# kaist-cvml/3d-vlm-gd

Hardware: AMD Instinct MI355X
Metric: image-pairs/sec (518^2, ViT-B/14 LoRA) student distillation step (higher is better)
Workload: dtype tf32h; 1 GPU; finetune_timm_mast3r_objaverse: vit_base/14 + LoRA(r=4,q,v)+adapters blocks 4-11, 518^2 pairs, shared-518 geometry, mast3r losses (AP+depth+intra+cost-KL), 32 pairs/GPU, 300 keypoints/pair, hw=1369; pairs_per_gpu=32, global_pairs=32, parallelism=dp1, world_size_seen=1, backend=nccl (RCCL), exchange=torch, engine_dtype=tf32h

## Files before the change

### 3d-vlm-gd_amd/_lib.py

```python
import ctypes
import os

_HERE = os.path.dirname(os.path.abspath(__file__))
LIB_PATH = os.environ.get("GD_HIP_LIB") or os.path.join(_HERE, "lib", "libgd_hip.so")
_lib = None

F32, BF16, F16 = 0, 1, 3
MATCH_COLS = 1

c_int, c_long, c_float, c_void_p, c_size_t = ctypes.c_int, ctypes.c_long, ctypes.c_float, ctypes.c_void_p, ctypes.c_size_t

ABI_VERSION = 4
SIGNATURES = {
    "gd_last_error": (ctypes.c_char_p, []),
    "gd_abi_version": (c_int, []),
    "gd_debug_set": (c_int, [ctypes.c_char_p, c_int]),
    "gd_debug_get": (c_int, [ctypes.c_char_p]),
    "gd_gemm_phase_probe": (c_int, [c_int, c_void_p]),
    "gd_loss_combine_fwd": (c_int, [c_void_p, c_void_p, c_void_p, c_void_p, ctypes.POINTER(c_float), c_void_p, c_int, c_void_p, c_void_p, c_void_p]),
    "gd_loss_combine_bwd": (c_int, [c_void_p, ctypes.POINTER(c_float), c_void_p, c_int, c_void_p, c_void_p]),
    "gd_depth_bwd_combine": (c_int, [c_void_p, c_void_p, c_void_p, c_void_p, c_void_p, c_void_p, c_int, c_int, c_int, c_void_p, c_void_p, c_void_p]),
    "gd_scale_and_transpose": (c_int, [c_void_p, c_void_p, c_void_p, c_void_p, c_int, c_int, c_int, c_void_p]),
    "gd_gemm_nt": (c_int, [c_void_p, c_void_p, c_void_p, c_int, c_int, c_int, c_long, c_long, c_long,
                           c_int, c_long, c_long, c_long, c_int, c_int, c_float,
# ... 10 lines not shown
                                           c_int, c_int, c_int, c_int, c_void_p, c_void_p, c_void_p, c_void_p]),
    "gd_cost_volume_kl_bwd_rows_workspace_bytes": (c_size_t, [c_int, c_int, c_int, c_int, c_int]),
    "gd_cost_volume_kl_bwd_rows": (c_int, [c_void_p, c_void_p, c_void_p, c_void_p, c_void_p, c_void_p, c_int, c_void_p, c_void_p, c_int, c_int, c_int,
                                           c_int, c_int, c_void_p, c_void_p, c_void_p, c_void_p, c_void_p, c_void_p]),
    "gd_cost_volume_kl_bwd_h_workspace_bytes": (c_size_t, [c_int, c_int, c_int]),
    "gd_cost_volume_kl_bwd_h": (c_int, [c_void_p, c_void_p, c_void_p, c_void_p, c_void_p, c_void_p, c_int, c_void_p, c_void_p, c_int, c_int, c_int,
                                        c_void_p, c_void_p, c_void_p, c_void_p, c_void_p, c_void_p]),
    "gd_gemm_nt_copy16": (c_int, [c_void_p, c_void_p, c_void_p, c_int, c_int, c_int, c_long, c_long, c_long, c_float, c_void_p, c_void_p,
                                  c_void_p, c_long, c_void_p, c_long, c_void_p, c_void_p]),
    "gd_tap_mean_norm_fwd_h": (c_int, [c_void_p, c_int, c_long, c_int, c_void_p, c_void_p, c_void_p, c_int, c_int, c_int, c_void_p]),
    "gd_adapter_fused_h_supported": (c_int, [c_int, c_int, c_long]),
    "gd_adapter_fused_h_ln": (c_int, [c_void_p, c_void_p, c_void_p, c_void_p, c_void_p, c_void_p, c_void_p, c_float, c_void_p, c_void_p, c_void_p,
                                      c_int, c_int, c_int, c_void_p]),
    "gd_adapter_fused_h": (c_int, [c_void_p, c_void_p, c_void_p, c_void_p, c_void_p, c_void_p, c_void_p, c_void_p, c_void_p, c_void_p,
                                   c_int, c_int, c_int, c_void_p]),
    "gd_gemm_tn_scaled": (c_int, [c_void_p, c_void_p, c_void_p, c_int, c_int, c_int, c_long, c_long, c_long,
                                  c_int, c_long, c_long, c_long, c_int, c_int, c_float, c_void_p, c_void_p]),
    "gd_cast_f16": (c_int, [c_void_p, c_void_p, c_long, c_int, c_long, c_float, c_void_p, c_void_p]),
    "gd_amax_scale": (c_int, [c_void_p, c_long, c_int, c_long, c_float, c_void_p, c_void_p, c_void_p]),
    "gd_scale_from_amax": (c_int, [c_void_p, c_float, c_void_p, c_void_p]),
    "gd_cast_f16_ex": (c_int, [c_void_p, c_void_p, c_long, c_int, c_long, c_float, c_void_p, c_void_p, c_void_p]),
    "gd_layernorm_bwd_ex": (c_int, [c_void_p, c_int, c_void_p, c_void_p, c_void_p, c_void_p, c_void_p, c_void_p, c_void_p, c_void_p, c_void_p, c_void_p,
                                    c_void_p, c_void_p, c_int, c_int, c_long, c_long, c_float, c_void_p]),
    "gd_gemm_tn": (c_int, [c_void_p, c_void_p, c_void_p, c_int, c_int, c_int, c_long, c_long, c_long,
                           c_int, c_long, c_long, c_long, c_int, c_int, c_float, c_void_p]),
    "gd_layernorm_fwd": (c_int, [c_void_p, c_void_p, c_void_p, c_void_p, c_void_p, c_void_p, c_int, c_int, c_long,
                                 c_long, c_float, c_int, c_int, c_void_p]),
    "gd_layernorm_bwd": (c_int, [c_void_p, c_void_p, c_void_p, c_void_p, c_void_p, c_void_p, c_void_p, c_void_p, c_int, c_int,
                                 c_long, c_long, c_float, c_int, c_int, c_void_p]),
    "gd_adapter_fused_supported": (c_int, [c_int, c_int, c_int]),
    "gd_adapter_fused": (c_int, [c_void_p, c_void_p, c_void_p, c_void_p, c_void_p, c_void_p, c_int, c_int, c_int, c_int,
                                 c_void_p]),
    "gd_l2norm_fwd": (c_int, [c_void_p, c_void_p, c_void_p, c_int, c_int, c_float, c_void_p]),
    "gd_l2norm_bwd": (c_int, [c_void_p, c_void_p, c_void_p, c_void_p, c_int, c_int, c_void_p]),
    "gd_patch_im2col": (c_int, [c_void_p, c_void_p, c_int, c_int, c_int, c_int, c_int, c_int, c_int,
                                ctypes.POINTER(c_float), ctypes.POINTER(c_float), c_int, c_void_p]),
    "gd_patch_im2col_strided": (c_int, [c_void_p, c_void_p, c_int, c_int, c_int, c_int, c_int, c_int, c_int, c_int, c_int,
                                        ctypes.POINTER(c_float), ctypes.POINTER(c_float), c_int, c_void_p]),
    "gd_assemble_tokens": (c_int, [c_void_p, c_void_p, c_void_p, c_void_p, c_int, c_int, c_int, c_int, c_void_p]),
    "gd_im2col3x3": (c_int, [c_void_p, c_long, c_void_p, c_int, c_int, c_int, c_int, c_int, c_void_p]),
    "gd_col2im3x3": (c_int, [c_void_p, c_void_p, c_long, c_int, c_int, c_int, c_int, c_int, c_void_p]),
    "gd_kp_gather_fwd": (c_int, [ctypes.POINTER(c_void_p), c_int, c_long, c_int, c_void_p, c_void_p, c_int, c_int,
                                 c_int, c_int, c_int, c_float, c_float, c_int, c_int, c_int, c_int, c_int, c_void_p]),
    "gd_kp_gather_fwd_ln": (c_int, [ctypes.POINTER(c_void_p), ctypes.POINTER(c_void_p), ctypes.POINTER(c_void_p), c_int, c_long, c_long, c_int, c_void_p, c_void_p,
                                    c_void_p, c_void_p, c_int, c_int, c_int, c_int, c_int, c_float, c_float, c_int, c_int, c_int, c_int, c_int, c_void_p]),
    "gd_kp_gather_bwd": (c_int, [ctypes.POINTER(c_void_p), c_int, c_long, c_void_p, c_void_p, c_int, c_int, c_int, c_int,
# ... 156 lines not shown
```

### 3d-vlm-gd_amd/csrc/norm.hip

```cpp
#include "gd_common.h"
#include <stdlib.h>

#define LN_MAXV 8

template <typename T> __device__ __forceinline__ f32x4 load4(const T* p);
template <> __device__ __forceinline__ f32x4 load4<float>(const float* p) { return *(const f32x4*)p; }
template <> __device__ __forceinline__ f32x4 load4<bf16>(const bf16* p) {
    const bf16x4 v = *(const bf16x4*)p;
    return f32x4{(float)v[0], (float)v[1], (float)v[2], (float)v[3]};
}
template <typename T> __device__ __forceinline__ void store4n(T* p, f32x4 v);
template <> __device__ __forceinline__ void store4n<float>(float* p, f32x4 v) { *(f32x4*)p = v; }
template <> __device__ __forceinline__ void store4n<bf16>(bf16* p, f32x4 v) {
    *(bf16x4*)p = bf16x4{(bf16)v[0], (bf16)v[1], (bf16)v[2], (bf16)v[3]};
}
template <> __device__ __forceinline__ void store4n<f16>(f16* p, f32x4 v) {
    *(f16x4*)p = f16_sat4(v[0], v[1], v[2], v[3]);
}

template <typename T, typename TO, int NV>
__global__ __launch_bounds__(256) void ln_fwd_kernel(const T* x, const float* gamma, const float* beta, TO* y,
                                                     float* mean, float* rstd, int M, int D, long ldx, long ldy,
                                                     float eps) {
    const int lane = threadIdx.x & 63, row = blockIdx.x * 4 + (threadIdx.x >> 6);
// ... 32 lines not shown
            for (int k = 0; k < 4; ++k) o[k] = (v[i][k] - mu) * rs * g[k] + b[k];
            store4n<TO>(yr + c, o);
        }
    }
}

template <> __device__ __forceinline__ f32x4 load4<f16>(const f16* p) {
    const f16x4 v = *(const f16x4*)p;
    return f32x4{(float)v[0], (float)v[1], (float)v[2], (float)v[3]};
}
__device__ __forceinline__ unsigned wave_umax(unsigned v) {
#pragma unroll
    for (int o = 32; o > 0; o >>= 1) { const unsigned w = (unsigned)__shfl_xor((int)v, o, 64); v = w > v ? w : v; }
    return v;
}
__device__ __forceinline__ unsigned wave_uadd(unsigned v) {
#pragma unroll
    for (int o = 32; o > 0; o >>= 1) v += (unsigned)__shfl_xor((int)v, o, 64);
    return v;
}
#define GD_AMAX_SLOTS 256
#define GD_RANGE_SLOTS 64

template <typename T, typename TD, int NV>
__global__ __launch_bounds__(256) void ln_bwd_kernel(const TD* dy, const T* x, const float* gamma, const float* mean,
                                                     const float* rstd, const T* dres, const T* dres2, T* dx, int M, int D,
                                                     long ldd, long ldx, float dyscale, f16* dx16 = nullptr, const float* sdev = nullptr,
                                                     const float* dys_dev = nullptr, unsigned* amax = nullptr, unsigned* range = nullptr) {
    const int lane = threadIdx.x & 63;
    int row = blockIdx.x * 4 + (threadIdx.x >> 6);
    const bool live = row < M;
    if (!live) {
        if (!amax && !range) return;
        row = M - 1;
    }
    const float mu = mean[row], rs = rstd[row];
    const float s16 = (dx16 && sdev) ? *sdev : 1.0f;
    if (dys_dev) dyscale *= *dys_dev;
    const T* xr = x + (long)row * ldx;
    const TD* dr = dy + (long)row * ldd;
    f32x4 xh[NV], g[NV];
    float s1 = 0.f, s2 = 0.f;
    unsigned mb = 0u, nsat = 0u, nlow = 0u;
#pragma unroll
    for (int i = 0; i < NV; ++i) {
        const int c = (lane + 64 * i) * 4;
        if (c < D) {
            const f32x4 xv = load4<T>(xr + c), dv = load4<TD>(dr + c), gm = *(const f32x4*)(gamma + c);
#pragma unroll
            for (int k = 0; k < 4; ++k) {
                xh[i][k] = (xv[k] - mu) * rs;
                g[i][k] = dv[k] * dyscale * gm[k];
                s1 += g[i][k];
                s2 += g[i][k] * xh[i][k];
            }
            if (sizeof(TD) == 2 && sizeof(T) == 4 && range && live) {
#pragma unroll
                for (int k = 0; k < 4; ++k) nsat += !(fabsf(dv[k]) < 65504.0f);
            }
        }
    }
    s1 = wave_sum(s1) / (float)D;
    s2 = wave_sum(s2) / (float)D;
    T* or_ = dx + (long)row * ldx;
#pragma unroll
    for (int i = 0; i < NV; ++i) {
        const int c = (lane + 64 * i) * 4;
        if (c < D) {
            f32x4 o;
#pragma unroll
            for (int k = 0; k < 4; ++k) o[k] = rs * (g[i][k] - s1 - xh[i][k] * s2);
            if (dres) {
                const f32x4 r = load4<T>(dres + (long)row * ldx + c);
#pragma unroll
                for (int k = 0; k < 4; ++k) o[k] += r[k];
            }
            if (dres2) {
                const f32x4 r = load4<T>(dres2 + (long)row * ldx + c);
#pragma unroll
                for (int k = 0; k < 4; ++k) o[k] += r[k];
            }
            if (live) store4n<T>(or_ + c, o);
            if (amax) {
#pragma unroll
                for (int k = 0; k < 4; ++k) { const unsigned b = gd_f2u(o[k]) & 0x7fffffffu; mb = b > mb ? b : mb; }
            }
            if (dx16) {
                const f32x4 os = o * s16;
                if (live) store4n<f16>(dx16 + (long)row * D + c, os);
                if (range && live) {
#pragma unroll
                    for (int k = 0; k < 4; ++k) {
                        const unsigned b = gd_f2u(os[k]) & 0x7fffffffu;
                        nsat += b > 0x477fe000u;
                        nlow += (b < 0x38800000u) & (b != 0u);
                    }
                }
            }
        }
    }
    if (amax || range) {
        __shared__ unsigned red[3][4];
        const int w = threadIdx.x >> 6;
        if (amax) mb = wave_umax(mb);
        if (range) { nsat = wave_uadd(nsat); nlow = wave_uadd(nlow); }
// ... 211 lines not shown
    hipStream_t s = (hipStream_t)stream;
#define B_FH(NV) hipLaunchKernelGGL((ln_bwd_kernel<float, float, NV>), grid, blk, 0, s, dy, x, gamma, mean, rstd, dres, dres2, dx, M, D, ldd, ldx, dyscale, (f16*)dx16, scale_dev)
    LN_DISPATCH_NV(D, B_FH);
    GD_LAUNCH_OK();
    return 0;
}

extern "C" int gd_layernorm_bwd_ex(const void* dy, int dy_dtype, const float* dy_scale_dev, const float* x, const float* gamma, const float* mean,
                                   const float* rstd, const float* dres, const float* dres2, float* dx, void* dx16, const float* cast_scale_dev,
                                   unsigned* amax_slots, unsigned* range_counters, int M, int D, long ldd, long ldx, float dyscale, void* stream) {
    GD_REQUIRE(M > 0 && D > 0 && D % 4 == 0 && D <= 64 * 4 * LN_MAXV, "gd_layernorm_bwd_ex: D=%d must be a multiple of 4 and <= 2048", D);
    GD_REQUIRE(ldx % 4 == 0 && ldd % 4 == 0, "gd_layernorm_bwd_ex: row strides must be multiples of 4 elements");
    GD_REQUIRE(dy_dtype == GD_F32 || dy_dtype == GD_F16, "gd_layernorm_bwd_ex: dy is f32 or fp16 (dy_dtype %d)", dy_dtype);
    GD_REQUIRE(((uintptr_t)dy & 7) == 0 && ((uintptr_t)x & 15) == 0 && ((uintptr_t)dx & 15) == 0, "gd_layernorm_bwd_ex: alignment");
    dim3 grid(gd_cdiv(M, 4)), blk(256);
    hipStream_t s = (hipStream_t)stream;
#define B_XF(NV) hipLaunchKernelGGL((ln_bwd_kernel<float, float, NV>), grid, blk, 0, s, (const float*)dy, x, gamma, mean, rstd, dres, dres2, dx, M, D, ldd, ldx, dyscale, (f16*)dx16, cast_scale_dev, dy_scale_dev, amax_slots, range_counters)
#define B_XH(NV) hipLaunchKernelGGL((ln_bwd_kernel<float, f16, NV>), grid, blk, 0, s, (const f16*)dy, x, gamma, mean, rstd, dres, dres2, dx, M, D, ldd, ldx, dyscale, (f16*)dx16, cast_scale_dev, dy_scale_dev, amax_slots, range_counters)
    if (dy_dtype == GD_F16) LN_DISPATCH_NV(D, B_XH); else LN_DISPATCH_NV(D, B_XF);
    GD_LAUNCH_OK();
    return 0;
}

extern "C" int gd_l2norm_fwd(const float* x, float* y, float* inv, int M, int D, float eps, void* stream) {
    GD_REQUIRE(M > 0 && D > 0, "gd_l2norm_fwd: bad shape");
    hipLaunchKernelGGL(l2norm_fwd_kernel, dim3(gd_cdiv(M, 4)), dim3(256), 0, (hipStream_t)stream, x, y, inv, M, D, eps);
    GD_LAUNCH_OK();
    return 0;
}
extern "C" int gd_l2norm_bwd(const float* y, const float* dy, const float* inv, float* dx, int M, int D, void* stream) {
    GD_REQUIRE(M > 0 && D > 0, "gd_l2norm_bwd: bad shape");
    hipLaunchKernelGGL(l2norm_bwd_kernel, dim3(gd_cdiv(M, 4)), dim3(256), 0, (hipStream_t)stream, y, dy, inv, dx, M, D);
    GD_LAUNCH_OK();
    return 0;
}
```

### 3d-vlm-gd_amd/ops.py

```python
import torch

from . import _lib
from ._lib import check, dtype_code, lib, ptr, stream
from .options import option


def _req(cond, msg):
    if not cond:
        raise _lib.GdHipError(msg)


class GemmProfiler:

    def __init__(self):
        self.records = []

    def totals(self, keep=None):
        torch.cuda.synchronize()
        recs = [r for r in self.records if keep is None or keep(r[3])]
        flops = sum(r[2] for r in recs)
        ms = sum(r[0].elapsed_time(r[1]) for r in recs)
        return flops, ms, len(recs)

    def roofline_time(self, keep, peak_flops, peak_bytes):
# ... 491 lines not shown
    _req(x32.dtype == torch.float32 and x32.is_contiguous() and w1.dtype == torch.float16 and w2.dtype == torch.float16 and w1.is_contiguous() and
         w2.is_contiguous() and w1.shape == (bott, D) and w2.shape == (D, bott) and ln_w.dtype == torch.float32 and ln_b.dtype == torch.float32, "adapter_fused_h_ln: layout")
    out = torch.empty_like(x32)
    hidden = torch.empty(M, bott, dtype=torch.float16, device=x32.device)
    y16 = torch.empty(M, D, dtype=torch.float16, device=x32.device)
    mean = torch.empty(M, dtype=torch.float32, device=x32.device)
    rstd = torch.empty(M, dtype=torch.float32, device=x32.device)
    check(lib().gd_adapter_fused_h_ln(ptr(x32), ptr(w1), ptr(w2), ptr(hidden), ptr(out), ptr(ln_w), ptr(ln_b), float(ln_eps), ptr(y16), ptr(mean), ptr(rstd),
                                      M, D, bott, stream()), "gd_adapter_fused_h_ln")
    return out, hidden, y16, mean, rstd


def layernorm_fwd(x, gamma, beta, eps, *, save_stats=True, out_dtype=None):
    M, D = x.shape
    y = torch.empty(M, D, dtype=out_dtype or x.dtype, device=x.device)
    mean = torch.empty(M, dtype=torch.float32, device=x.device) if save_stats else None
    rstd = torch.empty(M, dtype=torch.float32, device=x.device) if save_stats else None
    rc = lib().gd_layernorm_fwd(ptr(x), ptr(gamma), ptr(beta), ptr(y), ptr(mean), ptr(rstd), M, D, x.stride(0),
                                y.stride(0), float(eps), dtype_code(x), dtype_code(y), stream())
    check(rc, "gd_layernorm_fwd")
    return y, mean, rstd


def layernorm_bwd(dy, x, gamma, mean, rstd, dres=None, dyscale=1.0, dres2=None, cast_scale=None, dy_scale=None, want_amax=False):
    M, D = x.shape
    if cast_scale is not None or dy_scale is not None or want_amax or dy.dtype == torch.float16:
        _req(x.is_contiguous() and x.dtype == torch.float32 and dy.dtype in (torch.float32, torch.float16) and dy.stride(-1) == 1 and
             all(t is None or (t.is_contiguous() and t.dtype == x.dtype and t.numel() == x.numel()) for t in (dres, dres2)),
             "layernorm_bwd (tf32h form): fp32 x / dres, fp32 or fp16 dy, contiguous")
        dx = torch.empty_like(x)
        dx16 = torch.empty(M, D, dtype=torch.float16, device=x.device) if cast_scale is not None else None
        slots = _slots(x.device) if want_amax else None
        rng = _RANGE if ((dx16 is not None or dy.dtype == torch.float16) and _RANGE is not None and _RANGE.device == x.device) else None
        check(lib().gd_layernorm_bwd_ex(ptr(dy), dtype_code(dy), ptr(dy_scale), ptr(x), ptr(gamma), ptr(mean), ptr(rstd), ptr(dres), ptr(dres2), ptr(dx),
                                        ptr(dx16), ptr(cast_scale), ptr(slots), ptr(rng), M, D, dy.stride(0), x.stride(0), float(dyscale), stream()),
              "gd_layernorm_bwd_ex")
        if want_amax:
            sc = torch.empty(3, dtype=torch.float32, device=x.device)
            check(lib().gd_scale_from_amax(ptr(slots), GRAD_TARGET, ptr(sc), stream()), "gd_scale_from_amax")
            amax_register(dx, sc)
        return (dx, dx16) if cast_scale is not None else dx
    _req(x.is_contiguous() and dy.stride(-1) == 1 and all(t is None or (t.is_contiguous() and t.dtype == x.dtype and
                                                                        t.numel() == x.numel()) for t in (dres, dres2)),
         "layernorm_bwd: layout")
    dx = torch.empty_like(x)
    rc = lib().gd_layernorm_bwd(ptr(dy), ptr(x), ptr(gamma), ptr(mean), ptr(rstd), ptr(dres), ptr(dres2), ptr(dx), M, D,
                                dy.stride(0), x.stride(0), float(dyscale), dtype_code(x), dtype_code(dy), stream())
    check(rc, "gd_layernorm_bwd")
# ... 837 lines not shown
```

### 3d-vlm-gd_amd/options.py

```python
import os

_DEFS = {
    "conv_at_kp": ("GD_CONV_AT_KP", 1),
    "conv_dx_at_kp": ("GD_CONV_DX_AT_KP", 1),
    "conv_stacked": ("GD_CONV_STACKED", 1),
    "lora_fused": ("GD_LORA_FUSED", 1),
    "gather_det": ("GD_GATHER_DET", 1),
    "adapter_h_fused": ("GD_ADAPTER_H_FUSED", 1),
    "cv_bwd_rows": ("GD_CV_BWD_ROWS", 1),
    "h16_dy": ("GD_H16_DY", 1),
    "tap_norm_fused": ("GD_TAP_NORM_FUSED", 1),
    "adapter_ln": ("GD_ADAPTER_LN", 1),
    "direct_grads": ("GD_DIRECT_GRADS", 1),
}
_VALUES = {k: int(os.environ.get(env, str(d))) for k, (env, d) in _DEFS.items()}


def option(name):
    return _VALUES[name]


def set_option(name, value):
    if name not in _VALUES:
        raise KeyError(f"unknown option {name!r}: {sorted(_VALUES)}")
    old = _VALUES[name]
    _VALUES[name] = int(value)
    return old
```

### 3d-vlm-gd_amd/vit.py

```python
import math

import torch
import torch.nn as nn
import torch.nn.functional as F

from . import ops
from .options import option
from .model import Adapter, BlockWithAdapter, _LoRA_qkv


def _dt(name):
    return {"f32": torch.float32, "bf16": torch.bfloat16, "tf32x": torch.float32, "tf32h": torch.float32, torch.float32: torch.float32,
            torch.bfloat16: torch.bfloat16}[name]


def _opa(x, fmt, sc=None):
    return ops.split3(x, "a") if fmt == "x3" else ops.cast16(x, scale_dev=None if sc is None else sc[0:1])


def _opw(w, fmt):
    return ops.split3(w, "w") if fmt == "x3" else ops.cast16(w)


LORA_B_SHIFT = 12
# ... 272 lines not shown
                if fmt == "h" and ops.copy16_ok(dhpa.shape[0], D, dhpa.shape[1]):
                    dx2, dx2a = ops.gemm_nt_copy16(dhpa, w_dt, dout.view(-1, D), alpha_dev=ad, copy_scale=sc[0:1])
                else:
                    dx2 = ops.gemm_nt(dhpa, w_dt, residual=dout.view(-1, D), out_dtype=torch.float32, alpha_dev=ad)
            else:
                dhp = ops.gemm_nt(dout, up_tT, dact_src=hd, dact=2)
                dx2 = ops.gemm_nt(dhp, down_tT, residual=dout)
            if ad_h:
                pass
            elif fmt == "h" and ctx.hd16 is not None and x2.dtype == torch.float16:
                g_up = ops.gemm_tn(douta, ctx.hd16, out=z_up, alpha_dev=sc[1:2])
                g_down = ops.gemm_tn(dhpa, x2, out=z_down, alpha_dev=sc[1:2])
                del douta, dhpa
            else:
                g_up = ops.gemm_tn(dout, hd, out=z_up)
                g_down = ops.gemm_tn(dhp, x2, out=z_down)
        hs = bool(fmt) and ops.split_out_ok(dx2.shape[0], plan["w2_t"].shape[0], plan["w2_t"].shape[1]) and (fmt != "h" or pre.dtype == torch.float16)
        hkw = {} if not hs else {"out_split": True} if fmt == "x3" else {"out_dtype": torch.float16}
        dpre = _mm(dx2, plan, "w2_t", xs=dx2a, sc=sc, dact_src=pre, dact=3, **hkw)
        h16dy = fmt == "h" and hs and bool(option("h16_dy"))
        dy2 = _mm(None if hs else dpre, plan, "w1_t", xs=dpre if hs else None, sc=sc, **({"out_dtype": torch.float16} if h16dy else {}))
        del dpre
        if fmt == "h":
            dx1, dx1h = ops.layernorm_bwd(dy2, x1, plan["ln2_w"], mean2, rstd2, dres=dx2, cast_scale=sc[0:1], dy_scale=sc[1:2] if h16dy else None)
            do = _mm(None, plan, "wproj_t", xs=dx1h, sc=sc, out_dtype=torch.float16)
            del dx1h
        else:
            dx1 = ops.layernorm_bwd(dy2, x1, plan["ln2_w"], mean2, rstd2, dres=dx2)
            do = _mm(dx1, plan, "wproj_t", sc=sc)
        dqkv = ops.attention_bwd(qkv, o, do, lse, B, Nt, H, vfirst=True, need_dk=bool(ctx.needs_input_grad[0]), x3=fmt == "x3")
        if ctx.has_lora:
            r = at.shape[0] // 2
            bt_T = tw["bt_T"] if tw is not None else bt.to(T).contiguous()
            bt_qv = tw["bt_qv"] if tw is not None else torch.cat([bt_T[:, :D], bt_T[:, 2 * D:]], 1).contiguous()
            dqv = dqkv[:, :2 * D]
            gat = None
            dt_is_scaled = False
            if fmt == "h" and sc is not None and y1.dtype == torch.float16 and ops.lora_bwd_fused_h_supported(dqv, t, None, z_bt):
                bt16, dtm = (tw["bt_qv_w3"], tw["bt_qv_mul"]) if tw is not None and "bt_qv_w3" in tw and tw["bt_qv_w3"].dtype == torch.float16 \
                    else _opw_lora_b(bt_qv.float().contiguous())
                dt = ops.lora_bwd_fused_h(dqv, t, bt16, z_bt, out_mul=sc[1:2], dt_scaled=h16dy, dt_mul=dtm)
                gbt = z_bt
                if ops.lora_bwd_fused_h_supported(y1, dt, None, z_at):
                    sd = ops.amax_scale(dt, LORA_DT_TARGET)
                    ops.lora_bwd_fused_h(y1, dt, None, z_at, t_mul=sd[0:1], out_mul=sd[1:2] * sc[1:2] if h16dy else sd[1:2])
                else:
                    ops.gemm_tn(dt, y1, out=z_at, alpha_dev=sc[1:2] if h16dy else None)
# ... 25 lines not shown
                gbt = ops.gemm_tn(t, dqv, out=z_bt)
            if gat is not None:
                pass
            else:
                if ops.lora_bwd_fused_supported(y1, dt, None, z_at):
                    gat = ops.skinny_tn_mfma(dt, y1, z_at)
                else:
                    gat = ops.gemm_tn(dt, y1, out=z_at)
            g_bq, g_bv = gbt[:r, :D].t(), gbt[r:, D:].t()
            g_aq, g_av = gat[:r], gat[r:]
        if direct:
            g_aq = g_bq = g_av = g_bv = g_down = g_up = None
            if ctx.gate is not None:
                ctx.gate.node_done()
        if not ctx.needs_input_grad[0]:
            return None, None, None, None, g_aq, g_bq, g_av, g_bv, g_down, g_up
        if ctx.has_lora:
            h16dy1 = h16dy and dt_is_scaled
            dy1 = _mm(dqkv, plan, "wqkv_t_qvk", xs=dqkv_s if fmt else None, sc=sc, lora_t=dt, lora_b=at.contiguous(),
                      **({"out_dtype": torch.float16} if h16dy1 else {}))
        else:
            h16dy1 = h16dy and dqkv.dtype == torch.float16
            dy1 = _mm(dqkv, plan, "wqkv_t_qvk", xs=dqkv if dqkv.dtype == torch.float16 else None, sc=sc, **({"out_dtype": torch.float16} if h16dy1 else {}))
        if fmt == "h":
            dx = ops.layernorm_bwd(dy1, x, plan["ln1_w"], mean1, rstd1, dres=dx1, dy_scale=sc[1:2] if dy1.dtype == torch.float16 else None, want_amax=True)
        else:
            dx = ops.layernorm_bwd(dy1, x, plan["ln1_w"], mean1, rstd1, dres=dx1)
        return dx, None, None, None, g_aq, g_bq, g_av, g_bv, g_down, g_up


def run_block(blk, x, offer_ln_stats=False, next_block=None):
    inner, lora, adapter = _unwrap(blk)
    B, Nt, D = x.shape
    plan = inner.plan(x.dtype)
    a_q = b_q = a_v = b_v = down = up = None
    if lora is not None:
        if lora.linear_a_k is not None or lora.linear_a_v is None:
            raise ops._lib.GdHipError("the fused LoRA epilogue implements the reference's q+v configuration")
        a_q, b_q = lora.linear_a_q.weight, lora.linear_b_q.weight
        a_v, b_v = lora.linear_a_v.weight, lora.linear_b_v.weight
        if 2 * a_q.shape[0] > 8:
            raise ops._lib.GdHipError("LoRA rank > 4 not supported by the fused epilogue")
    if adapter is not None:
        down, up = adapter.down.weight, adapter.up.weight
    tw = getattr(inner, "_tw", None)
    if tw is not None and tw.get("dtype") == x.dtype:
        plan = dict(plan, tw=tw)
    if offer_ln_stats:
        plan = dict(plan, offer_ln_stats=True)
    if next_block is not None and adapter is not None and plan["x3"] == "h" and bool(option("adapter_ln")):
        pn = _unwrap(next_block)[0].plan(x.dtype)
        plan = dict(plan, next_ln=(pn["ln1_w"], pn["ln1_b"], pn["eps1"]))
    out = _BlockFn.apply(x.reshape(B * Nt, D), plan, B, Nt, a_q, b_q, a_v, b_v, down, up)
    return out.view(B, Nt, D)


class _LNFn(torch.autograd.Function):
    @staticmethod
    def forward(ctx, x, w, b, eps):
        shp = x.shape
        x2 = x.reshape(-1, shp[-1]).contiguous()
        wf, bf = w.detach().float().contiguous(), b.detach().float().contiguous()
        y, mean, rstd = ops.layernorm_fwd(x2, wf, bf, eps, save_stats=x.requires_grad)
        if x.requires_grad:
            ctx.save_for_backward(x2, wf, mean, rstd)
            ctx.shp = shp
        return y.view(shp)

    @staticmethod
    def backward(ctx, dy):
        x2, wf, mean, rstd = ctx.saved_tensors
        dy2 = dy.reshape(-1, dy.shape[-1]).contiguous()
# ... 12 lines not shown
        ctx.amax = bool(amax)
        x2 = x.reshape(-1, shp[-1]).contiguous()
        wf, bf = w.detach().float().contiguous(), b.detach().float().contiguous()
        if defer is not None:
            defer.update(x2=x2, w=wf, b=bf, eps=float(eps))
            ctx.defer = defer
            ctx.save_for_backward(x2, wf)
            ctx.shp = shp
            return x.view_as(x), x.view_as(x), x.view_as(x)
        ctx.defer = None
        y, mean, rstd = ops.layernorm_fwd(x2, wf, bf, eps, save_stats=x.requires_grad, out_dtype=out_dtype)
        if x.requires_grad:
            ctx.save_for_backward(x2, wf, mean, rstd)
            ctx.shp = shp
        return x.view_as(x), x.view_as(x), y.view(shp)

    @staticmethod
    def backward(ctx, g_next, g_raw, g_norm):
        if ctx.defer is not None:
            x2, wf = ctx.saved_tensors
            mean, rstd = deferred_stats(ctx.defer)
        else:
            x2, wf, mean, rstd = ctx.saved_tensors
        if g_next is not None:
            ops.amax_take(g_next)
        res = [g.reshape(x2.shape).contiguous().to(x2.dtype) for g in (g_next, g_raw) if g is not None]
        if g_norm is None:
            dx = None if not res else (res[0] if len(res) == 1 else res[0] + res[1])
        else:
            dy = g_norm.reshape(x2.shape).contiguous()
            if dy.dtype not in (torch.float32, x2.dtype) or (x2.dtype == torch.float32 and dy.dtype != torch.float32):
                dy = dy.float()
            dx = ops.layernorm_bwd(dy, x2, wf, mean, rstd, dres=res[0] if res else None,
                                   dres2=res[1] if len(res) > 1 else None, want_amax=ctx.amax and x2.dtype == torch.float32)
        return (dx.view(ctx.shp) if dx is not None else None), None, None, None, None, None, None


def deferred_stats(defer):
    if "mean" not in defer:
        _, defer["mean"], defer["rstd"] = ops.layernorm_fwd(defer["x2"], defer["w"], defer["b"], defer["eps"], save_stats=True)
    return defer["mean"], defer["rstd"]


class _DeferredNormFn(torch.autograd.Function):

    @staticmethod
    def forward(ctx, t, rec):
        return ops.layernorm_fwd(rec["x2"], rec["w"], rec["b"], rec["eps"], save_stats=False)[0].view(t.shape)

    @staticmethod
    def backward(ctx, dy):
        return dy, None


class DeferredTapNorm:
    __slots__ = ("raw", "rec")

    def __init__(self, raw, rec):
        self.raw, self.rec = raw, rec

    shape = property(lambda self: self.raw.shape)
    dtype = property(lambda self: self.raw.dtype)
    device = property(lambda self: self.raw.device)

    def materialize(self):
        return _DeferredNormFn.apply(self.raw, self.rec)


class GDLayerNorm(nn.LayerNorm):

    def forward(self, x):
        return _LNFn.apply(x, self.weight, self.bias, self.eps)


class GDPatchEmbed(nn.Module):
    def __init__(self, patch_size, in_chans, embed_dim, bias=True):
        super().__init__()
        self.patch_size = (patch_size, patch_size)
        self.proj = nn.Conv2d(in_chans, embed_dim, kernel_size=patch_size, stride=patch_size, bias=bias)


VIT_PRESETS = {
    "vit_tiny_test": (64, 8, 1), "vit_small": (384, 12, 6), "vit_base": (768, 12, 12), "vit_large": (1024, 24, 16),
}


class GDViT(nn.Module):

# ... 209 lines not shown
        x = self.embed(x, size)
        outs = []
        for i, blk in enumerate(self.blocks):
            x = run_block(blk, x)
            if i in take:
                outs.append(x)
        return outs

    def forward_features(self, x, size=None):
        x = self.embed(x, size)
        for blk in self.blocks:
            x = run_block(blk, x)
        return self.norm(x)

    def forward_all(self, x, taps, size=None, norm_taps=False):
        ops.ln_stats_clear()
        x = self.embed(x, size)
        outs, normed = {}, {}
        pending = None
        defer_ok = (norm_taps == "deferred" and bool(option("tap_norm_fused")) and torch.is_grad_enabled() and self.tap_norm_dtype is None
                    and (self.embed_dim * (2 if self.dtype == torch.bfloat16 else 4)) % 16 == 0)
        for i, blk in enumerate(self.blocks):
            x_in = x
            x = run_block(blk, x, offer_ln_stats=pending is not None, next_block=self.blocks[i + 1] if i + 1 < len(self.blocks) else None)
            if pending is not None:
                st = ops.ln_stats_take(x_in.reshape(-1, x_in.shape[-1]), pending["eps"])
                if st is not None:
                    pending["mean"], pending["rstd"] = st
                pending = None
            if i in taps:
                if norm_taps and i + 1 < len(self.blocks):
                    rec = {} if (defer_ok and x.requires_grad) else None
                    x, outs[i], normed[i] = _TapFn.apply(x, self.norm.weight, self.norm.bias, self.norm.eps, self.tap_norm_dtype, self.opfmt == "h", rec)
                    if rec is not None:
                        inner = _unwrap(self.blocks[i + 1])[0]
                        if inner.norm1.eps == self.norm.eps:
                            pending = rec
                        normed[i] = DeferredTapNorm(normed[i], rec)
                else:
                    outs[i] = x
                    if norm_taps:
                        normed[i] = self.norm(x)
        if norm_taps:
            return [outs[i] for i in taps], x, [normed[i] for i in taps]
        return [outs[i] for i in taps], x

    def forward(self, x):
# ... 186 lines not shown
```

### include/gd_hip.h

```cpp
#ifndef GD_HIP_H
#define GD_HIP_H
#include <stddef.h>
#ifdef __cplusplus
extern "C" {
#endif

#define GD_F32 0
#define GD_BF16 1
#define GD_F32X3 2
#define GD_F16 3

const char* gd_last_error(void);
#define GD_ABI_VERSION 4
int gd_abi_version(void);

int gd_debug_set(const char* name, int value);
int gd_debug_get(const char* name);
int gd_gemm_phase_probe(int enable, unsigned long long* out6);

int gd_gemm_nt(const void* A, const void* W, void* C, int M, int N, int K, long lda, long ldw, long ldc,
               int batch, long sA, long sW, long sC, int ab_dtype, int c_dtype, float alpha,
               const float* bias, const float* lora_t, const float* lora_b, int lora_rt, void* preact, long ldp,
               int act, const void* dact_src, long ldd, int dact, const void* residual, long ldr, int accumulate,
               void* stream);
// ... 164 lines not shown
                            const unsigned char* m1, const unsigned char* m2, int P, int hw, int C, const float* gloss, const float* stats,
                            float* df1, float* df2, void* workspace, void* stream);
int gd_gemm_nt_copy16(const void* A, const void* W, void* C, int M, int N, int K, long lda, long ldw, long ldc, float alpha,
                      const float* alpha_dev, const float* bias, const void* residual, long ldr, void* copy16, long ldc16,
                      const float* copy_scale_dev, void* stream);
int gd_gemm_tn_scaled(const void* Y, const void* X, float* G, int M, int N, int K, long ldy, long ldx, long ldg,
                      int batch, long sY, long sX, long sG, int y_dtype, int x_dtype, float alpha, const float* alpha_dev, void* stream);
int gd_adapter_fused_h_supported(int D, int bottleneck, long M);
int gd_adapter_fused_h_ln(const float* x32, const void* w1, const void* w2, void* hidden, float* out32, const float* ln_w, const float* ln_b,
                          float ln_eps, void* ln16, float* ln_mean, float* ln_rstd, int M, int D, int bottleneck, void* stream);
int gd_adapter_fused_h(const float* x32, const void* w1, const void* w2, const void* gate_src, void* hidden, float* out32, void* out16,
                       const float* in_scale, const float* alpha_dev, const float* copy_scale, int M, int D, int bottleneck, void* stream);
int gd_tap_mean_norm_fwd_h(const void* const* grids, int ngrid, long bstride, int prefix, float* out, void* out16, float* inv_norm,
                           int B, int hw, int D, void* stream);
int gd_layernorm_bwd_cast(const float* dy, const float* x, const float* gamma, const float* mean, const float* rstd,
                          const float* dres, const float* dres2, float* dx, void* dx16, const float* scale_dev, int M, int D,
                          long ldd, long ldx, float dyscale, void* stream);
int gd_amax_scale(const float* in, long rows, int K, long ld_in, float target, float* scale3, unsigned* amax_slots, void* stream);
int gd_scale_from_amax(unsigned* amax_slots, float target, float* scale2, void* stream);
int gd_cast_f16_ex(const float* in, void* out, long rows, int K, long ld_in, float scale, const float* scale_dev, unsigned* range_counters, void* stream);
int gd_layernorm_bwd_ex(const void* dy, int dy_dtype, const float* dy_scale_dev, const float* x, const float* gamma, const float* mean,
                        const float* rstd, const float* dres, const float* dres2, float* dx, void* dx16, const float* cast_scale_dev,
                        unsigned* amax_slots, unsigned* range_counters, int M, int D, long ldd, long ldx, float dyscale, void* stream);
int gd_gemm_nt_scaled(const void* A, const void* W, void* C, int M, int N, int K, long lda, long ldw, long ldc,
                      int batch, long sA, long sW, long sC, int ab_dtype, int c_dtype, float alpha, const float* alpha_dev,
                      const float* bias, const float* lora_t, const float* lora_b, int lora_rt, void* preact, long ldp,
                      int act, const void* dact_src, long ldd, int dact, const void* residual, long ldr, int accumulate,
                      void* stream);

int gd_comm_rccl_version(void);
int gd_comm_unique_id(void* out128);
int gd_comm_init(void** comm, int nranks, int rank, const void* id128);
int gd_comm_destroy(void* comm);
int gd_flat_allreduce(void* comm, float* buf, long n, int nranks, int rank, int algo, void* stream);

int gd_unproject_depth(const float* depth, const float* extrinsic, const float* intrinsic, float* out, int S, int H,
                       int W, void* stream);
int gd_coview_masks(const float* pm1, const float* pm2, const float* K1, const float* E1, const float* K2,
                    const float* E2, unsigned char* m1, unsigned char* m2, int P, int H, int W, void* stream);
int gd_nms_keypoints(const unsigned char* mask, const float* conf, int min_distance, unsigned char* keep_ws, int* idx,
                     int* count, int P, int H, int W, int cap, void* stream);
int gd_nn_argmax(const float* queries, const float* database, const unsigned char* active, int* idx,
                 unsigned long long* key_ws, int Nq, int Nb, int D, void* stream);
int gd_point_cloud_to_depth(const float* points, const float* K, float* depth, float* cnt_ws, int P, int Np, int w,
                            int h, void* stream);

// ... 52 lines not shown
```

Measured before the change: 550.6 image-pairs/s.

## Merge block LayerNorm-1 backward with tap norm backward into one dual-LN kernel

```diff
diff --git a/3d-vlm-gd_amd/_lib.py b/3d-vlm-gd_amd/_lib.py
--- a/3d-vlm-gd_amd/_lib.py
+++ b/3d-vlm-gd_amd/_lib.py
@@ -56,6 +56,9 @@
     "gd_cast_f16_ex": (c_int, [c_void_p, c_void_p, c_long, c_int, c_long, c_float, c_void_p, c_void_p, c_void_p]),
     "gd_layernorm_bwd_ex": (c_int, [c_void_p, c_int, c_void_p, c_void_p, c_void_p, c_void_p, c_void_p, c_void_p, c_void_p, c_void_p, c_void_p, c_void_p,
                                     c_void_p, c_void_p, c_int, c_int, c_long, c_long, c_float, c_void_p]),
+    "gd_layernorm_bwd_dual": (c_int, [c_void_p, c_int, c_void_p, c_void_p, c_void_p, c_void_p, c_void_p, c_void_p, c_void_p, c_void_p, c_void_p, c_int,
+                                      c_int, c_float, c_void_p, c_void_p, c_void_p, c_void_p, c_void_p, c_int, c_int, c_long, c_long, c_long, c_float,
+                                      c_void_p]),
     "gd_gemm_tn": (c_int, [c_void_p, c_void_p, c_void_p, c_int, c_int, c_int, c_long, c_long, c_long,
                            c_int, c_long, c_long, c_long, c_int, c_int, c_float, c_void_p]),
     "gd_layernorm_fwd": (c_int, [c_void_p, c_void_p, c_void_p, c_void_p, c_void_p, c_void_p, c_int, c_int, c_long,
diff --git a/3d-vlm-gd_amd/csrc/norm.hip b/3d-vlm-gd_amd/csrc/norm.hip
--- a/3d-vlm-gd_amd/csrc/norm.hip
+++ b/3d-vlm-gd_amd/csrc/norm.hip
@@ -78,11 +78,13 @@
 #define GD_AMAX_SLOTS 256
 #define GD_RANGE_SLOTS 64
 
-template <typename T, typename TD, int NV>
+template <typename T, typename TD, int NV, bool DUAL = false, bool EXT = false>
 __global__ __launch_bounds__(256) void ln_bwd_kernel(const TD* dy, const T* x, const float* gamma, const float* mean,
                                                      const float* rstd, const T* dres, const T* dres2, T* dx, int M, int D,
                                                      long ldd, long ldx, float dyscale, f16* dx16 = nullptr, const float* sdev = nullptr,
-                                                     const float* dys_dev = nullptr, unsigned* amax = nullptr, unsigned* range = nullptr) {
+                                                     const float* dys_dev = nullptr, unsigned* amax = nullptr, unsigned* range = nullptr,
+                                                     const float* dy_b = nullptr, const float* gamma_b = nullptr, long ldd_b = 0,
+                                                     int map_hw = 0, int map_prefix = 0, float map_scale = 1.0f) {
     const int lane = threadIdx.x & 63;
     int row = blockIdx.x * 4 + (threadIdx.x >> 6);
     const bool live = row < M;
@@ -107,8 +109,19 @@
             for (int k = 0; k < 4; ++k) {
                 xh[i][k] = (xv[k] - mu) * rs;
                 g[i][k] = dv[k] * dyscale * gm[k];
-                s1 += g[i][k];
-                s2 += g[i][k] * xh[i][k];
+                if constexpr (!DUAL) {
+                    s1 += g[i][k];
+                    s2 += g[i][k] * xh[i][k];
+                }
+            }
+            if constexpr (DUAL) {
+                const f32x4 bv = *(const f32x4*)(dy_b + (long)row * ldd_b + c), gb = *(const f32x4*)(gamma_b + c);
+#pragma unroll
+                for (int k = 0; k < 4; ++k) {
+                    g[i][k] += bv[k] * gb[k];
+                    s1 += g[i][k];
+                    s2 += g[i][k] * xh[i][k];
+                }
             }
             if (sizeof(TD) == 2 && sizeof(T) == 4 && range && live) {
 #pragma unroll
@@ -119,6 +132,15 @@
     s1 = wave_sum(s1) / (float)D;
     s2 = wave_sum(s2) / (float)D;
     T* or_ = dx + (long)row * ldx;
+    const T* r2 = nullptr;
+    if constexpr (EXT) {
+        if (dres2 && map_hw > 0) {
+            const int nt = map_prefix + map_hw, b = row / nt, r = row - b * nt;
+            if (r >= map_prefix) r2 = dres2 + ((long)b * map_hw + (r - map_prefix)) * D;
+        } else if (dres2) {
+            r2 = dres2 + (long)row * ldx;
+        }
+    }
 #pragma unroll
     for (int i = 0; i < NV; ++i) {
         const int c = (lane + 64 * i) * 4;
@@ -131,12 +153,21 @@
 #pragma unroll
                 for (int k = 0; k < 4; ++k) o[k] += r[k];
             }
-            if (dres2) {
-                const f32x4 r = load4<T>(dres2 + (long)row * ldx + c);
-#pragma unroll
-                for (int k = 0; k < 4; ++k) o[k] += r[k];
-            }
-            if (live) store4n<T>(or_ + c, o);
+            if constexpr (EXT) {
+                if (r2) {
+                    const f32x4 r = load4<T>(r2 + c);
+#pragma unroll
+                    for (int k = 0; k < 4; ++k) o[k] += map_hw > 0 ? r[k] * map_scale : r[k];
+                }
+                if (live && dx) store4n<T>(or_ + c, o);
+            } else {
+                if (dres2) {
+                    const f32x4 r = load4<T>(dres2 + (long)row * ldx + c);
+#pragma unroll
+                    for (int k = 0; k < 4; ++k) o[k] += r[k];
+                }
+                if (live) store4n<T>(or_ + c, o);
+            }
             if (amax) {
 #pragma unroll
                 for (int k = 0; k < 4; ++k) { const unsigned b = gd_f2u(o[k]) & 0x7fffffffu; mb = b > mb ? b : mb; }
@@ -394,6 +425,36 @@
     return 0;
 }
 
+extern "C" int gd_layernorm_bwd_dual(const void* dy, int dy_dtype, const float* dy_scale_dev, const float* dy_b, const float* gamma_b, const float* x,
+                                     const float* gamma, const float* mean, const float* rstd, const float* dres, const float* dres2, int map_hw,
+                                     int map_prefix, float map_scale, float* dx, void* dx16, const float* cast_scale_dev, unsigned* amax_slots,
+                                     unsigned* range_counters, int M, int D, long ldd, long ldd_b, long ldx, float dyscale, void* stream) {
+    GD_REQUIRE(M > 0 && D > 0 && D % 4 == 0 && D <= 64 * 4 * LN_MAXV, "gd_layernorm_bwd_dual: D=%d must be a multiple of 4 and <= 2048", D);
+    GD_REQUIRE(ldx % 4 == 0 && ldd % 4 == 0 && ldx >= D && ldd >= D, "gd_layernorm_bwd_dual: row strides must be multiples of 4 elements, at least D");
+    GD_REQUIRE(dy_dtype == GD_F32 || dy_dtype == GD_F16, "gd_layernorm_bwd_dual: dy is f32 or fp16 (dy_dtype %d)", dy_dtype);
+    GD_REQUIRE(dy && x && gamma && mean && rstd, "gd_layernorm_bwd_dual: dy, x, gamma, mean, rstd required");
+    GD_REQUIRE(dx != nullptr || dx16 != nullptr, "gd_layernorm_bwd_dual: dx may be null only when dx16 is given");
+    GD_REQUIRE((dy_b == nullptr) == (gamma_b == nullptr), "gd_layernorm_bwd_dual: dy_b and gamma_b come together");
+    GD_REQUIRE(dy_b == nullptr || (ldd_b % 4 == 0 && ldd_b >= D && ((uintptr_t)dy_b & 15) == 0 && ((uintptr_t)gamma_b & 15) == 0),
+               "gd_layernorm_bwd_dual: dy_b rows are 16-byte aligned multiples of 4 elements, at least D");
+    GD_REQUIRE(map_hw >= 0 && map_prefix >= 0, "gd_layernorm_bwd_dual: map_hw=%d, map_prefix=%d must not be negative", map_hw, map_prefix);
+    GD_REQUIRE(map_hw == 0 || (dres2 != nullptr && M % (map_prefix + map_hw) == 0),
+               "gd_layernorm_bwd_dual: a mapped dres2 needs M=%d to be whole images of map_prefix + map_hw rows", M);
+    GD_REQUIRE(((uintptr_t)dy & 7) == 0 && ((uintptr_t)x & 15) == 0 && ((uintptr_t)dx & 15) == 0 && ((uintptr_t)dres & 15) == 0 &&
+               ((uintptr_t)dres2 & 15) == 0 && ((uintptr_t)dx16 & 7) == 0 && ((uintptr_t)gamma & 15) == 0, "gd_layernorm_bwd_dual: alignment");
+    dim3 grid(gd_cdiv(M, 4)), blk(256);
+    hipStream_t s = (hipStream_t)stream;
+#define B_DARGS x, gamma, mean, rstd, dres, dres2, dx, M, D, ldd, ldx, dyscale, (f16*)dx16, cast_scale_dev, dy_scale_dev, amax_slots, range_counters, dy_b, gamma_b, ldd_b, map_hw, map_prefix, map_scale
+#define B_DF0(NV) hipLaunchKernelGGL((ln_bwd_kernel<float, float, NV, false, true>), grid, blk, 0, s, (const float*)dy, B_DARGS)
+#define B_DF1(NV) hipLaunchKernelGGL((ln_bwd_kernel<float, float, NV, true, true>), grid, blk, 0, s, (const float*)dy, B_DARGS)
+#define B_DH0(NV) hipLaunchKernelGGL((ln_bwd_kernel<float, f16, NV, false, true>), grid, blk, 0, s, (const f16*)dy, B_DARGS)
+#define B_DH1(NV) hipLaunchKernelGGL((ln_bwd_kernel<float, f16, NV, true, true>), grid, blk, 0, s, (const f16*)dy, B_DARGS)
+    if (dy_dtype == GD_F16) { if (dy_b) LN_DISPATCH_NV(D, B_DH1); else LN_DISPATCH_NV(D, B_DH0); }
+    else { if (dy_b) LN_DISPATCH_NV(D, B_DF1); else LN_DISPATCH_NV(D, B_DF0); }
+    GD_LAUNCH_OK();
+    return 0;
+}
+
 extern "C" int gd_l2norm_fwd(const float* x, float* y, float* inv, int M, int D, float eps, void* stream) {
     GD_REQUIRE(M > 0 && D > 0, "gd_l2norm_fwd: bad shape");
     hipLaunchKernelGGL(l2norm_fwd_kernel, dim3(gd_cdiv(M, 4)), dim3(256), 0, (hipStream_t)stream, x, y, inv, M, D, eps);
diff --git a/3d-vlm-gd_amd/ops.py b/3d-vlm-gd_amd/ops.py
--- a/3d-vlm-gd_amd/ops.py
+++ b/3d-vlm-gd_amd/ops.py
@@ -537,8 +537,37 @@
     return y, mean, rstd
 
 
-def layernorm_bwd(dy, x, gamma, mean, rstd, dres=None, dyscale=1.0, dres2=None, cast_scale=None, dy_scale=None, want_amax=False):
+def layernorm_bwd(dy, x, gamma, mean, rstd, dres=None, dyscale=1.0, dres2=None, cast_scale=None, dy_scale=None, want_amax=False, dy2=None,
+                  gamma2=None, dres2_map=None, want_dx=True):
     M, D = x.shape
+    if dy2 is not None or dres2_map is not None or not want_dx:
+        _req(x.is_contiguous() and x.dtype == torch.float32 and dy.dtype in (torch.float32, torch.float16) and dy.stride(-1) == 1 and
+             (dres is None or (dres.is_contiguous() and dres.dtype == x.dtype and dres.numel() == x.numel())),
+             "layernorm_bwd (dual form): fp32 x / dres, fp32 or fp16 dy, contiguous")
+        _req((dy2 is None) == (gamma2 is None) and (dy2 is None or (dy2.dtype == torch.float32 and dy2.shape == x.shape and dy2.stride(-1) == 1 and
+                                                                  gamma2.dtype == torch.float32 and gamma2.is_contiguous() and gamma2.numel() == D)),
+             "layernorm_bwd (dual form): dy2 [M, D] fp32 comes with gamma2 [D] fp32")
+        _req(want_dx or (cast_scale is not None and not want_amax), "layernorm_bwd: want_dx=False needs cast_scale (dx16 is the result) and carries no amax")
+        hw = prefix = 0
+        mscale = 1.0
+        if dres2_map is not None:
+            prefix, hw, mscale = int(dres2_map[0]), int(dres2_map[1]), float(dres2_map[2])
+            _req(dres2 is not None and dres2.is_contiguous() and dres2.dtype == x.dtype and hw > 0 and prefix >= 0 and M % (prefix + hw) == 0 and
+                 dres2.numel() == M // (prefix + hw) * hw * D, "layernorm_bwd: a mapped dres2 is [M / (prefix + hw), hw, D]")
+        else:
+            _req(dres2 is None or (dres2.is_contiguous() and dres2.dtype == x.dtype and dres2.numel() == x.numel()), "layernorm_bwd (dual form): dres2 layout")
+        dx = torch.empty_like(x) if want_dx else None
+        dx16 = torch.empty(M, D, dtype=torch.float16, device=x.device) if cast_scale is not None else None
+        slots = _slots(x.device) if want_amax else None
+        rng = _RANGE if ((dx16 is not None or dy.dtype == torch.float16) and _RANGE is not None and _RANGE.device == x.device) else None
+        check(lib().gd_layernorm_bwd_dual(ptr(dy), dtype_code(dy), ptr(dy_scale), ptr(dy2), ptr(gamma2), ptr(x), ptr(gamma), ptr(mean), ptr(rstd), ptr(dres),
+                                          ptr(dres2), hw, prefix, mscale, ptr(dx), ptr(dx16), ptr(cast_scale), ptr(slots), ptr(rng), M, D, dy.stride(0),
+                                          dy2.stride(0) if dy2 is not None else 0, x.stride(0), float(dyscale), stream()), "gd_layernorm_bwd_dual")
+        if want_amax:
+            sc = torch.empty(3, dtype=torch.float32, device=x.device)
+            check(lib().gd_scale_from_amax(ptr(slots), GRAD_TARGET, ptr(sc), stream()), "gd_scale_from_amax")
+            amax_register(dx, sc)
+        return (dx, dx16) if cast_scale is not None else dx
     if cast_scale is not None or dy_scale is not None or want_amax or dy.dtype == torch.float16:
         _req(x.is_contiguous() and x.dtype == torch.float32 and dy.dtype in (torch.float32, torch.float16) and dy.stride(-1) == 1 and
              all(t is None or (t.is_contiguous() and t.dtype == x.dtype and t.numel() == x.numel()) for t in (dres, dres2)),
diff --git a/3d-vlm-gd_amd/options.py b/3d-vlm-gd_amd/options.py
--- a/3d-vlm-gd_amd/options.py
+++ b/3d-vlm-gd_amd/options.py
@@ -11,6 +11,7 @@
     "h16_dy": ("GD_H16_DY", 1),
     "tap_norm_fused": ("GD_TAP_NORM_FUSED", 1),
     "adapter_ln": ("GD_ADAPTER_LN", 1),
+    "tap_ln1_merge": ("GD_TAP_LN1_MERGE", 1),
     "direct_grads": ("GD_DIRECT_GRADS", 1),
 }
 _VALUES = {k: int(os.environ.get(env, str(d))) for k, (env, d) in _DEFS.items()}
diff --git a/3d-vlm-gd_amd/vit.py b/3d-vlm-gd_amd/vit.py
--- a/3d-vlm-gd_amd/vit.py
+++ b/3d-vlm-gd_amd/vit.py
@@ -318,7 +318,8 @@
         dy2 = _mm(None if hs else dpre, plan, "w1_t", xs=dpre if hs else None, sc=sc, **({"out_dtype": torch.float16} if h16dy else {}))
         del dpre
         if fmt == "h":
-            dx1, dx1h = ops.layernorm_bwd(dy2, x1, plan["ln2_w"], mean2, rstd2, dres=dx2, cast_scale=sc[0:1], dy_scale=sc[1:2] if h16dy else None)
+            dx1, dx1h = ops.layernorm_bwd(dy2, x1, plan["ln2_w"], mean2, rstd2, dres=dx2, cast_scale=sc[0:1], dy_scale=sc[1:2] if h16dy else None,
+                                          want_dx=bool(ctx.needs_input_grad[0]) or not option("tap_ln1_merge"))
             do = _mm(None, plan, "wproj_t", xs=dx1h, sc=sc, out_dtype=torch.float16)
             del dx1h
         else:
@@ -390,6 +391,13 @@
         else:
             h16dy1 = h16dy and dqkv.dtype == torch.float16
             dy1 = _mm(dqkv, plan, "wqkv_t_qvk", xs=dqkv if dqkv.dtype == torch.float16 else None, sc=sc, **({"out_dtype": torch.float16} if h16dy1 else {}))
+        rec = plan.get("tap_rec")
+        if (rec is not None and bool(option("tap_ln1_merge")) and x.dtype == torch.float32 and not rec.get("materialized")
+                and rec.get("mean") is not None and rec["mean"].data_ptr() == mean1.data_ptr() and rec["rstd"].data_ptr() == rstd1.data_ptr()):
+            if "ln1_pending" in rec:
+                raise RuntimeError("_BlockFn.backward: the LayerNorm-1 term left for the tap below was never taken by its backward")
+            rec["ln1_pending"] = (dy1, sc[1:2] if dy1.dtype == torch.float16 else None, plan["ln1_w"])
+            return dx1, None, None, None, g_aq, g_bq, g_av, g_bv, g_down, g_up
         if fmt == "h":
             dx = ops.layernorm_bwd(dy1, x, plan["ln1_w"], mean1, rstd1, dres=dx1, dy_scale=sc[1:2] if dy1.dtype == torch.float16 else None, want_amax=True)
         else:
@@ -397,7 +405,7 @@
         return dx, None, None, None, g_aq, g_bq, g_av, g_bv, g_down, g_up
 
 
-def run_block(blk, x, offer_ln_stats=False, next_block=None):
+def run_block(blk, x, offer_ln_stats=False, next_block=None, tap_rec=None):
     inner, lora, adapter = _unwrap(blk)
     B, Nt, D = x.shape
     plan = inner.plan(x.dtype)
@@ -415,7 +423,7 @@
     if tw is not None and tw.get("dtype") == x.dtype:
         plan = dict(plan, tw=tw)
     if offer_ln_stats:
-        plan = dict(plan, offer_ln_stats=True)
+        plan = dict(plan, offer_ln_stats=True, tap_rec=tap_rec)
     if next_block is not None and adapter is not None and plan["x3"] == "h" and bool(option("adapter_ln")):
         pn = _unwrap(next_block)[0].plan(x.dtype)
         plan = dict(plan, next_ln=(pn["ln1_w"], pn["ln1_b"], pn["eps1"]))
@@ -474,6 +482,16 @@
             mean, rstd = deferred_stats(ctx.defer)
         else:
             x2, wf, mean, rstd = ctx.saved_tensors
+        pend = ctx.defer.pop("ln1_pending", None) if ctx.defer is not None else None
+        if pend is not None:
+            if g_next is None:
+                raise RuntimeError("_TapFn.backward: a LayerNorm-1 term is pending but no gradient arrived from the block that left it")
+            dy1, dy1_scale, ln1_w = pend
+            g_next, g_raw = (None if g is None else g.reshape(x2.shape).contiguous().to(x2.dtype) for g in (g_next, g_raw))
+            g_norm = None if g_norm is None else g_norm.reshape(x2.shape).contiguous().float()
+            dx = ops.layernorm_bwd(dy1, x2, ln1_w, mean, rstd, dres=g_next, dres2=g_raw, dy_scale=dy1_scale, want_amax=ctx.amax,
+                                   dy2=g_norm, gamma2=wf if g_norm is not None else None)
+            return dx.view(ctx.shp), None, None, None, None, None, None
         if g_next is not None:
             ops.amax_take(g_next)
         res = [g.reshape(x2.shape).contiguous().to(x2.dtype) for g in (g_next, g_raw) if g is not None]
@@ -516,6 +534,7 @@
     device = property(lambda self: self.raw.device)
 
     def materialize(self):
+        self.rec["materialized"] = True
         return _DeferredNormFn.apply(self.raw, self.rec)
 
 
@@ -771,7 +790,7 @@
                     and (self.embed_dim * (2 if self.dtype == torch.bfloat16 else 4)) % 16 == 0)
         for i, blk in enumerate(self.blocks):
             x_in = x
-            x = run_block(blk, x, offer_ln_stats=pending is not None, next_block=self.blocks[i + 1] if i + 1 < len(self.blocks) else None)
+            x = run_block(blk, x, offer_ln_stats=pending is not None, next_block=self.blocks[i + 1] if i + 1 < len(self.blocks) else None, tap_rec=pending)
             if pending is not None:
                 st = ops.ln_stats_take(x_in.reshape(-1, x_in.shape[-1]), pending["eps"])
                 if st is not None:
diff --git a/include/gd_hip.h b/include/gd_hip.h
--- a/include/gd_hip.h
+++ b/include/gd_hip.h
@@ -210,6 +210,10 @@
 int gd_layernorm_bwd_ex(const void* dy, int dy_dtype, const float* dy_scale_dev, const float* x, const float* gamma, const float* mean,
                         const float* rstd, const float* dres, const float* dres2, float* dx, void* dx16, const float* cast_scale_dev,
                         unsigned* amax_slots, unsigned* range_counters, int M, int D, long ldd, long ldx, float dyscale, void* stream);
+int gd_layernorm_bwd_dual(const void* dy, int dy_dtype, const float* dy_scale_dev, const float* dy_b, const float* gamma_b, const float* x,
+                          const float* gamma, const float* mean, const float* rstd, const float* dres, const float* dres2, int map_hw,
+                          int map_prefix, float map_scale, float* dx, void* dx16, const float* cast_scale_dev, unsigned* amax_slots,
+                          unsigned* range_counters, int M, int D, long ldd, long ldd_b, long ldx, float dyscale, void* stream);
 int gd_gemm_nt_scaled(const void* A, const void* W, void* C, int M, int N, int K, long lda, long ldw, long ldc,
                       int batch, long sA, long sW, long sC, int ab_dtype, int c_dtype, float alpha, const float* alpha_dev,
                       const float* bias, const float* lora_t, const float* lora_b, int lora_rt, void* preact, long ldp,
```

Measured after the change: 556.4 image-pairs/s (median of 6 runs). +1.1%, better.
